# edawson/rkmh

Measured on AMD Instinct MI355X. Metric: reads classified/sec, higher is better.
Workload: dtype u64; 1 GPU; stream (C2): 1000000 synthetic 150 bp reads per GPU vs data/all_pave_ref.fa (182 refs), k=16 s=1000; reads_per_gpu=1000000, read_len=150, k=16, sketch_size=1000, references=182, parallelism=reads sharded over 1 rank(s); ref sketches RCCL-broadcast once

## Files before the change

### rkmh_amd/csrc/rk_kmer.hip

```cpp
#include "rk_kernels.hpp"

#include <cstdlib>
#include <type_traits>

namespace rk {

namespace {

constexpr int KW = 64;
constexpr int KM_MAX_T = 8;
constexpr int KM_MQ = 32;
constexpr int KM_CH = 2;
constexpr int KM_QCAP = 64 + 4 * KW;
constexpr int KM_LDS_SMALL = 5120;
constexpr int KM_LDS_BIG = 20480;
constexpr int KM_WAVES = 8;

enum { CM_DENSE8 = 0, CM_DENSE16 = 1, CM_SPARSE = 2 };

struct KmerGeom {
    int32_t T;
    int32_t cwords;
    int32_t dset;
    int32_t xcd;
    int32_t nmin_cap;
    int32_t L;
    int32_t gpr[KM_MAX_KS];
    uint32_t magic[KM_MAX_KS];
};

typedef uint32_t u32x4 __attribute__((ext_vector_type(4)));
struct __attribute__((packed, aligned(1))) km_pair1 { uint32_t x, y; };
struct __attribute__((packed, aligned(4))) km_pair4 { uint32_t x, y; };

template <int NQ>
struct KmLds {
    static constexpr int PK = 0;
    static constexpr int INV = PK + NQ * 64 + 2;
    static constexpr int Q = INV + NQ * 32 + 2;
    static constexpr int MQ = Q + KM_QCAP;
    static constexpr int RI = MQ + 2 * KM_MQ;
    static constexpr int NZ = RI + 4 * (KM_MAX_T + 1);
    static constexpr int BEST = NZ + KM_MAX_T;
    static constexpr int FLAGS = BEST + KM_MAX_T;
    static constexpr int NWT = FLAGS + KM_MAX_T;
    static constexpr int FAM = NWT + KM_MAX_T;
    static constexpr int FAMF = FAM + 4 * KM_MAX_T;
    static constexpr int CNT = FAMF + KM_MAX_T;
    static_assert(RI % 4 == 0, "rinfo is read with 16-byte LDS loads");
    static_assert(CNT % 4 == 0, "the multisets are cleared with 16-byte LDS stores");
};
inline size_t km_lds_bytes(const KmerGeom& g, int nq) {
    return ((size_t)(nq == 1 ? KmLds<1>::CNT : KmLds<2>::CNT) + (size_t)g.T * (size_t)(g.cwords + g.dset)) * 4;
}

__device__ __forceinline__ void wave_sync() {
    __builtin_amdgcn_fence(__ATOMIC_RELEASE, "wavefront");
    __builtin_amdgcn_wave_barrier();
    __builtin_amdgcn_fence(__ATOMIC_ACQUIRE, "wavefront");
}
template <int CTRL>
__device__ __forceinline__ int dpp_i32(int v) { return __builtin_amdgcn_update_dpp(v, v, CTRL, 0xf, 0xf, false); }
__device__ __forceinline__ int row_max_i32(int v) {
    int t;
    t = dpp_i32<0xB1>(v); v = t > v ? t : v;
    t = dpp_i32<0x4E>(v); v = t > v ? t : v;
    t = dpp_i32<0x141>(v); v = t > v ? t : v;
    t = dpp_i32<0x140>(v); v = t > v ? t : v;
    return v;
}
__device__ __forceinline__ int half_row_max_i32(int v) {
    int t;
    t = dpp_i32<0xB1>(v); v = t > v ? t : v;
    t = dpp_i32<0x4E>(v); v = t > v ? t : v;
    t = dpp_i32<0x141>(v); v = t > v ? t : v;
    return v;
}

__device__ __forceinline__ uint32_t km_pack4_hi(uint32_t x, uint32_t& mism) {
    const uint32_t c = (x >> 1) & 0x03030303u;
    mism |= (x & 0xDFDFDFDFu) ^ __builtin_amdgcn_perm(0x47544341u, 0x47544341u, c);
    return c * 0x01041040u;
}
__device__ __forceinline__ uint32_t km_pack16(const u32x4& v, uint32_t& mism) {
    const uint32_t m0 = km_pack4_hi(v.x, mism), m1 = km_pack4_hi(v.y, mism), m2 = km_pack4_hi(v.z, mism), m3 = km_pack4_hi(v.w, mism);
    const uint32_t lo = __builtin_amdgcn_perm(m1, m0, 0x0c0c0703u);
    const uint32_t hi = __builtin_amdgcn_perm(m3, m2, 0x07030c0cu);
    return lo | hi;
}
__device__ __forceinline__ uint32_t km_nonzero4(uint32_t m) {
    const uint32_t y = (m | ((m & 0x7f7f7f7fu) + 0x7f7f7f7fu)) & 0x80808080u;
    return ((y >> 7) * 0x01020408u) >> 24;
}

template <int CMODE>
__device__ __forceinline__ uint32_t km_field_max(uint32_t x) {
    if constexpr (CMODE == CM_DENSE8) {
        const uint32_t m01 = max(x & 0xFFu, (x >> 8) & 0xFFu), m23 = max((x >> 16) & 0xFFu, x >> 24);
        return max(m01, m23);
    } else return max(x & 0xFFFFu, x >> 16);
}

template <int KT, int NQ, int CMODE, bool BIG, bool FAM>
__global__ __launch_bounds__(KW, BIG ? 2 : KM_WAVES) void k_classify_kmer(const uint8_t* __restrict__ bases, const uint32_t* __restrict__ offs,
                                                                              uint32_t nreads, int S, RefIndex ix, KmerSets ksets,
                                                                              int32_t* __restrict__ out4, DevPolicy pol, KmerGeom geo) {
    static_assert(KT == 0 || KT == 32 || (KT >= 4 && KT <= 16), "a k-mer packs into 32 bits; the core is the (k-3)-mer");
    constexpr bool WIDE = KT == 32;
    using L = KmLds<NQ>;
    __shared__ __attribute__((aligned(16))) uint32_t smem[(BIG ? KM_LDS_BIG : KM_LDS_SMALL) / 4];
    constexpr uint32_t PAD_P = NQ * 1024;
    constexpr uint32_t clg = CMODE == CM_DENSE8 ? 2 : 1, cbits = 32u >> clg, cmask = (1u << cbits) - 1u;
    uint32_t* const pk = smem + L::PK;
    uint32_t* const inv = smem + L::INV;
    uint32_t* const q = smem + L::Q;
    uint32_t* const mq = smem + L::MQ;
    uint4* const rinfo = reinterpret_cast<uint4*>(smem + L::RI);
    uint32_t* const nzero = smem + L::NZ;
    uint32_t* const best = smem + L::BEST;
    uint32_t* const flags = smem + L::FLAGS;
    uint32_t* const nwtot = smem + L::NWT;
    uint32_t* const fam = smem + L::FAM;
    uint32_t* const famf = smem + L::FAMF;
    uint32_t* const cnt = smem + L::CNT;
    const int T = geo.T;
    const uint32_t CW = (uint32_t)geo.cwords, DS = (uint32_t)geo.dset;
    uint32_t* const dset = cnt + (uint32_t)T * CW;
    const uint32_t ds_shift = 32u - (uint32_t)__builtin_ctz(DS);
    const int lane = threadIdx.x;

    for (uint32_t i = lane; i < ((uint32_t)T * CW) >> 2; i += KW) reinterpret_cast<uint4*>(cnt)[i] = make_uint4(0u, 0u, 0u, 0u);
    const uint32_t ntiles = (nreads + (uint32_t)T - 1) / (uint32_t)T;
    const uintptr_t gb = reinterpret_cast<uintptr_t>(bases);
    const uintptr_t safe_hi = (gb + (uintptr_t)offs[nreads] + 4u) & ~(uintptr_t)3;

    auto tile_reads = [&](uint32_t tl) -> int {
        const uint32_t r = tl * (uint32_t)T;
        return (int)((nreads - r) < (uint32_t)T ? (nreads - r) : (uint32_t)T);
    };
    auto load_offsets = [&](uint32_t tl, uint32_t& a_, uint32_t& b_, uint32_t& o_) {
        const uint32_t r = tl * (uint32_t)T;
        const int n = tile_reads(tl);
        a_ = offs[r];
        b_ = offs[r + (uint32_t)n];
        o_ = offs[r + (uint32_t)(lane <= n ? lane : n)];
    };
    u32x4 pf[NQ];
    auto fetch_tile = [&](uint32_t a_, uint32_t b_) {
        const uintptr_t first = gb + a_;
        const uintptr_t base16 = first & ~(uintptr_t)15;
        const uint32_t nbytes = (uint32_t)(first - base16) + (b_ - a_);
        uint32_t nq = (nbytes + 15u) >> 4;
        if (nq > (uint32_t)(NQ * KW)) nq = NQ * KW;
        const bool safe = base16 >= gb && base16 + 16u * (uintptr_t)nq <= safe_hi;
#pragma unroll
        for (int r = 0; r < NQ; ++r) {
            const uint32_t qi = (uint32_t)r * KW + (uint32_t)lane;
            u32x4 v = {0u, 0u, 0u, 0u};
            if (qi < nq) {
                const uintptr_t qa = base16 + 16u * (uintptr_t)qi;
                if (safe) {
                    typedef const u32x4 __attribute__((address_space(1))) * gq_t;
                    v = __builtin_nontemporal_load((gq_t)qa);
                }
                else {
                    uint32_t d[4];
#pragma unroll
                    for (int j = 0; j < 4; ++j) {
                        const uintptr_t da = qa + 4u * (uintptr_t)j;
                        d[j] = (da >= gb && da + 4u <= safe_hi) ? *reinterpret_cast<const uint32_t*>(da) : 0u;
                    }
                    v.x = d[0]; v.y = d[1]; v.z = d[2]; v.w = d[3];
                }
            }
            pf[r] = v;
        }
    };

    uint32_t tile = blockIdx.x;
    if (geo.xcd) { const uint32_t per = (gridDim.x + 7u) >> 3; tile = (blockIdx.x & 7u) * per + (blockIdx.x >> 3); }
    if (tile >= ntiles) return;
    uint32_t cur_a = 0, cur_b = 0, cur_o = 0;
    load_offsets(tile, cur_a, cur_b, cur_o);
    fetch_tile(cur_a, cur_b);
    {
        const uint32_t r0 = tile * (uint32_t)T;
        const uint32_t ta = (uint32_t)__builtin_amdgcn_readfirstlane((int)cur_a);
        const uint32_t tb = (uint32_t)__builtin_amdgcn_readfirstlane((int)cur_b);
        const uint32_t mis = (uint32_t)((gb + ta) & 15u);
        const uint32_t nbytes = mis + (tb - ta);
        const uint32_t o_next = (uint32_t)__shfl_down((int)cur_o, 1);
        const uint32_t len = o_next - cur_o;
        int Tn = tile_reads(tile);
        uint32_t nq = (nbytes + 15u) >> 4;
        if (nbytes > (uint32_t)(NQ * 1024)) {
            const int Tn0 = Tn;
            Tn = __popcll(__ballot(lane < Tn0 && o_next - ta + mis <= (uint32_t)(NQ * 1024)));
            if (lane >= Tn && lane < Tn0) reinterpret_cast<int4*>(out4)[r0 + lane] = make_int4(-2, 0, 0, 0);
            nq = NQ * KW;
        }

        constexpr int NKC = KT ? 1 : KM_MAX_KS;
        const int NK = KT ? 1 : ksets.n;
        uint32_t nw_all = 0;
        if (lane < Tn) {
#pragma unroll
            for (int j = 0; j < NKC; ++j) if (j < NK) nw_all += (uint32_t)num_windows((int)len, WIDE ? (int)ix.kpk : (KT ? KT : ksets.k[j]), pol.drop_last_window);
        }
        if constexpr (FAM) { if (lane < 4 * KM_MAX_T) fam[lane] = 0; }
        if (lane < KM_MAX_T) {
            nzero[lane] = 0; best[lane] = 0; nwtot[lane] = nw_all;
            if constexpr (FAM) famf[lane] = 0;
            flags[lane] = nw_all > (CMODE == CM_SPARSE ? 0x7FFu : cmask) ? 1u : 0u;
        }
        const uint32_t ulen = (uint32_t)__builtin_amdgcn_readfirstlane((int)len);
        const bool same_len = __ballot(lane < Tn && len != ulen) == 0ull;
        uint32_t mism = 0;
#pragma unroll
        for (int r = 0; r < NQ; ++r) {
            const uint32_t qi = (uint32_t)r * KW + (uint32_t)lane;
            uint32_t m = 0;
            pk[qi] = km_pack16(pf[r], m);
            if (qi < nq) mism |= m;
        }
        if (lane < 2) pk[NQ * KW + lane] = 0;
        const bool has_invalid = __ballot(mism != 0u) != 0ull;
        if (has_invalid) {
#pragma unroll
            for (int r = 0; r < NQ; ++r) {
                const uint32_t qi = (uint32_t)r * KW + (uint32_t)lane;
                uint32_t m0 = 0, m1 = 0, m2 = 0, m3 = 0;
                km_pack4_hi(pf[r].x, m0); km_pack4_hi(pf[r].y, m1); km_pack4_hi(pf[r].z, m2); km_pack4_hi(pf[r].w, m3);
                const uint32_t b16 = km_nonzero4(m0) | (km_nonzero4(m1) << 4) | (km_nonzero4(m2) << 8) | (km_nonzero4(m3) << 12);
                reinterpret_cast<uint16_t*>(inv)[qi] = (uint16_t)(qi < nq ? b16 : 0u);
            }
            if (lane < 2) inv[NQ * 32 + lane] = 0;
        }
        for (int kk = 0; kk < NK; ++kk) {
        const int k = WIDE ? (int)ix.kpk : (KT ? KT : ksets.k[kk]);
        const uint32_t KMASK = (WIDE || k == 16) ? 0xffffffffu : ((1u << (2 * k)) - 1u);
        const uint32_t CMASK = WIDE ? 0xffffffffu : (1u << (2 * (k - 3))) - 1u;
        const uint64_t KMASK64 = WIDE ? (1ull << (2 * k)) - 1ull : 0ull, CMASK64 = WIDE ? (1ull << (2 * (k - 3))) - 1ull : 0ull;
        const uint32_t KBITS = (1u << k) - 1u;
        const uint4* const kf4p = KT ? ix.kf4 : ksets.kf4[kk];
        const uint4* const km1p = KT ? ix.km1 : ksets.km1[kk];
        const uint32_t* const km1v = KT ? ix.km1_vals : ksets.km1_vals[kk];
        const uint32_t kf4_n = KT ? ix.kf4_n : ksets.kf4_n[kk], km1_b = KT ? ix.km1_b : ksets.km1_b[kk];
        wave_sync();
        uint32_t nw = 0, ng = 0;
        if (lane < Tn) { nw = (uint32_t)num_windows((int)len, k, pol.drop_last_window); ng = (nw + 3u) >> 2; }
        uint32_t gs = ng;
        gs += (uint32_t)__builtin_amdgcn_update_dpp(0, (int)gs, 0x111, 0xf, 0xf, true);
        gs += (uint32_t)__builtin_amdgcn_update_dpp(0, (int)gs, 0x112, 0xf, 0xf, true);
        gs += (uint32_t)__builtin_amdgcn_update_dpp(0, (int)gs, 0x114, 0xf, 0xf, true);
        const uint32_t NG = (uint32_t)__builtin_amdgcn_readlane((int)gs, KM_MAX_T - 1);
        if (lane <= KM_MAX_T) rinfo[lane] = make_uint4(cur_o - ta + mis, nw, gs - ng, 0u);
        {
            uint4* d4 = reinterpret_cast<uint4*>(dset);
            for (uint32_t i = lane; i < ((uint32_t)Tn * DS) >> 2; i += KW) d4[i] = make_uint4(0u, 0u, 0u, 0u);
        }
        wave_sync();

        const uint32_t nw_u = (uint32_t)num_windows((int)ulen, k, pol.drop_last_window), gpr_u = (nw_u + 3u) >> 2;
        const bool uniform = same_len && gpr_u >= 2u;
        uint32_t magic = 0;
        if (uniform) magic = ulen == (uint32_t)geo.L ? geo.magic[kk] : (uint32_t)__builtin_amdgcn_readfirstlane((int)(0xFFFFFFFFu / gpr_u + 1u));
        uint32_t magic_v = magic, dlen_v = ulen - 4u * gpr_u;
        asm volatile("" : "+v"(magic_v), "+v"(dlen_v));

        auto count_posting = [&](uint32_t t, uint32_t crow_b, uint32_t ref) -> uint32_t {
            uint32_t* crow = reinterpret_cast<uint32_t*>(reinterpret_cast<uint8_t*>(cnt) + crow_b);
            const uint32_t M1 = CW - 1u, key = ref + 1u;
            uint32_t idx = ((ref * 0x9E3779B1u) >> 16) & M1, probe = 0, c = 0;
            for (; probe <= M1; ++probe) {
                const uint32_t old = atomicCAS(&crow[idx], 0u, (key << 11) | 1u);
                if (old == 0u) { c = 1u; break; }
                if ((old >> 11) == key) { c = (atomicAdd(&crow[idx], 1u) & 0x7FFu) + 1u; break; }
                idx = (idx + 1u) & M1;
            }
            if (probe > M1) { flags[t] = 1; return 0u; }
            return (c << 16) + (0xFFFFu - ref);
        };
        auto add_posting = [&](uint32_t t, uint32_t crow_b, uint32_t ref) {
            if constexpr (CMODE == CM_SPARSE) {
                const uint32_t v = count_posting(t, crow_b, ref);
                if (v) atomicMax(&best[t], v);
            } else {
                const uint32_t sh = (ref << (5 - clg)) & (32u - cbits);
                const uint32_t woff = (ref >> clg) << 2;
                atomicAdd(reinterpret_cast<uint32_t*>(reinterpret_cast<uint8_t*>(cnt) + crow_b + woff), 1u << sh);
            }
        };
        uint32_t mqn = 0;
        auto process_mq = [&]() {
            wave_sync();
            const uint32_t g = (uint32_t)lane >> 4, sl = (uint32_t)lane & 15u;
            auto walk = [&](uint32_t tr, const uint32_t* lp, uint32_t hdr, const km_pair4& pm0) {
                const uint32_t t = tr & 0xFFu, n = hdr & 0xFFFFFFu, base = FAM ? hdr >> 24 : 0u;
                if (base) {
                    if ((tr >> 8) != 0u) return;
                    if (sl == 0) { atomicAdd(&fam[4u * t + ((base - 1u) >> 1)], 1u << (16u * ((base - 1u) & 1u))); famf[t] = 1u; }
                    for (uint32_t c0 = 0; c0 < n; c0 += 16) {
                        const uint32_t c = c0 + sl;
                        if (c < n) {
                            km_pair4 pm = pm0;
                            if (c0) pm = *reinterpret_cast<const km_pair4*>(lp + 1 + 2 * c);
                            const uint32_t sh = (pm.x << (5 - clg)) & (32u - cbits), woff = (pm.x >> clg) << 2;
                            atomicAdd(reinterpret_cast<uint32_t*>(reinterpret_cast<uint8_t*>(cnt) + __umul24(t, CW * 4u) + woff), (pm.y >> 31) ? 0u - (1u << sh) : 1u << sh);
                        }
                    }
                    return;
                }
                for (uint32_t c0 = 0; c0 < n; c0 += 16) {
                    const uint32_t c = c0 + sl;
                    uint32_t v = 0;
                    if (c < n) {
                        km_pair4 pm = pm0;
                        if (c0) pm = *reinterpret_cast<const km_pair4*>(lp + 1 + 2 * c);
                        if ((tr >> 8) < pm.y) {
                            if constexpr (CMODE == CM_SPARSE) v = count_posting(t, __umul24(t, CW * 4u), pm.x);
                            else add_posting(t, __umul24(t, CW * 4u), pm.x);
                        }
                    }
                    if constexpr (CMODE == CM_SPARSE) {
                        v = (uint32_t)row_max_i32((int)v);
                        if (sl == 0 && v) atomicMax(&best[t], v);
                    }
                }
            };
            uint32_t j = g;
            uint32_t tr = 0, n = 0;
            const uint32_t* lp = ix.kpost;
            km_pair4 pm0{0u, 0u};
            if (j < mqn) { tr = mq[2 * j]; lp = ix.kpost + mq[2 * j + 1]; n = lp[0]; pm0 = *reinterpret_cast<const km_pair4*>(lp + 1 + 2 * sl); }
            while (j < mqn) {
                const uint32_t jn = j + KW / 16;
                uint32_t trn = 0, nn = 0;
                const uint32_t* lpn = ix.kpost;
                km_pair4 pmn{0u, 0u};
                if (jn < mqn) { trn = mq[2 * jn]; lpn = ix.kpost + mq[2 * jn + 1]; nn = lpn[0]; pmn = *reinterpret_cast<const km_pair4*>(lpn + 1 + 2 * sl); }
                walk(tr, lp, n, pm0);
                j = jn; tr = trn; lp = lpn; n = nn; pm0 = pmn;
            }
            wave_sync();
            mqn = 0;
        };
        struct Cand { uint32_t key, t, y, key_hi; uint4 c; };
        const uint32_t km_r = WIDE ? 8u : 2u * (uint32_t)k - km1_b, km_vb1 = 32u - KM1_HB - km_r;
        const uint32_t km_vmask = (1u << (km_vb1 - 1u)) - 1u, km_rmask = (1u << km_r) - 1u, nref = (uint32_t)ix.nref;
        auto wide_probe = [&](const Cand& c, const uint4& b, uint32_t hop, uint3& res, bool& again) {
            const uint32_t want = (hop << KW_TAG) | (c.y & ((1u << KW_TAG) - 1u));
            const uint32_t cells[4] = {b.x, b.y, b.z, b.w};
            res = make_uint3(KW_VID_NONE, 0u, 0u);
#pragma unroll
            for (int q = 0; q < 4; ++q) {
                const uint32_t num = cells[q] & KW_EMPTY;
                if ((cells[q] >> (KW_IDBITS + 1)) == want && num != KW_EMPTY && res.x == KW_VID_NONE) {
                    const uint2 kk = ix.kkeys[num];
                    if (kk.x == c.key && (kk.y & 0xFFu) == c.key_hi) res = make_uint3(kk.y >> 8, 0u, num);
                }
            }
            again = res.x == KW_VID_NONE && ((b.w >> KW_IDBITS) & 1u) != 0u && c.t != 0xFFFFFFFFu;
        };
        auto lookup = [&](uint32_t e, uint32_t qn) -> Cand {
            Cand c;
            uint32_t ent = PAD_P | (8u << 12);
            if (e < qn) ent = q[e];
            const uint32_t P = ent & 4095u, t = ent >> 12;
            const km_pair1 w = *reinterpret_cast<const km_pair1*>(reinterpret_cast<const uint8_t*>(pk) + (P >> 2));
            const uint2 ri = *reinterpret_cast<const uint2*>(&rinfo[t]);
            c.t = P - ri.x < ri.y ? t : 0xFFFFFFFFu;
            if constexpr (WIDE) {
                const uint64_t x = (join64(w.x, w.y) >> ((P & 3u) << 1)) & KMASK64;
                const uint64_t r = packed_revcomp64(x, k);
                const uint64_t key = x < r ? x : r;
                c.key = (uint32_t)key; c.key_hi = (uint32_t)(key >> 32);
                c.y = (uint32_t)(kw_y(key, k) >> (2u * (uint32_t)k - km1_b - KW_TAG));
                c.c = km1p[c.y >> KW_TAG];
                return c;
            }
            const uint32_t x = __builtin_amdgcn_alignbit(w.y, w.x, (P & 3u) << 1) & KMASK;
            const uint32_t r = packed_revcomp(x, k);
            c.key = x < r ? x : r;
            c.key_hi = 0;
            c.y = km1_y(c.key, k);
            c.c = km1p[c.y >> km_r];
            return c;
        };
        auto match_cell = [&](const uint4& b, uint32_t wantsh) -> uint32_t {
            const uint32_t lim = 1u << km_vb1;
            return (b.x ^ wantsh) < lim ? b.x : ((b.y ^ wantsh) < lim ? b.y : ((b.z ^ wantsh) < lim ? b.z : ((b.w ^ wantsh) < lim ? b.w : 0xFFFFFFFFu)));
        };
        auto first_match = [&](const Cand& c, uint32_t& cell, bool& again) {
            cell = match_cell(c.c, (c.y & km_rmask) << km_vb1);
            again = (cell & km_vmask) == km_vmask && ((c.c.w >> (km_vb1 - 1u)) & 1u) != 0u && c.t != 0xFFFFFFFFu;
        };
        auto hop_load = [&](const Cand& c, uint32_t hop, bool again) -> u32x4 {
            u32x4 v = {0u, 0u, 0u, 0u};
            if (again) v = *reinterpret_cast<const u32x4*>(km1p + (((c.y >> km_r) + hop) & ((1u << km1_b) - 1u)));
            return v;
        };
        auto next_match = [&](const Cand& c, uint32_t hop, const u32x4& nv, uint32_t& cell, bool& again) {
            if (again) {
                const uint4 nb = make_uint4(nv.x, nv.y, nv.z, nv.w);
                cell = match_cell(nb, ((c.y & km_rmask) << km_vb1) | (hop << (32u - KM1_HB)));
                again = (cell & km_vmask) == km_vmask && ((nb.w >> (km_vb1 - 1u)) & 1u) != 0u;
            }
        };
        auto apply = [&](const Cand& c, uint32_t cell, uint3 wres = make_uint3(0u, 0u, 0u)) {
            uint32_t vid = cell & km_vmask;
            bool hit = vid != km_vmask && c.t != 0xFFFFFFFFu;
            bool zero = vid == km_vmask - 1u;
            if constexpr (WIDE) {
                vid = wres.x;
                hit = vid != KW_VID_NONE && c.t != 0xFFFFFFFFu;
                zero = vid == KW_VID_ZERO;
                if (hit && !zero && ix.keepkey) { const uint32_t kid = ix.kslots[wres.z]; if (!((ix.keepkey[kid >> 5] >> (kid & 31u)) & 1u)) zero = true; }
            }
            uint32_t val = vid | (1u << 20);
            uint32_t valy = 0, valz = 0, valw = 0;
            if (hit && vid >= nref && !zero) {
                const uint4 vv = *reinterpret_cast<const uint4*>(km1v + 4u * (vid - nref));
                val = vv.x; valy = vv.y; valz = vv.z; valw = vv.w;
                if constexpr (CMODE == CM_SPARSE) { if ((val >> 29) == 7u) val = 0x80000000u | valz; }
            }
            uint32_t rank = 0;
            bool multi = false;
            if (hit) {
                if (zero) atomicAdd(&nzero[c.t], 1u);
                else {
                    uint32_t* ds = dset + c.t * DS;
                    const uint32_t id = (WIDE ? wres.z : c.key) + 1u;
                    uint32_t idx = ((id - 1u) * 0x9E3779B1u) >> ds_shift;
                    uint32_t old = atomicCAS(&ds[idx], 0u, id);
                    uint32_t probes = 1;
                    while (old != 0u && probes < DS) {
                        rank += old == id ? 1u : 0u;
                        idx = (idx + 1u) & (DS - 1u);
                        old = atomicCAS(&ds[idx], 0u, id);
                        ++probes;
                    }
                    if (old != 0u) flags[c.t] = 1;
                    else if (FAM && (val >> 29) == 7u) {
                        if (rank == 0) {
                            const uint32_t base = (val >> 26) & 7u, nex = (val >> 22) & 15u, crow_b = __umul24(c.t, CW * 4u);
                            atomicAdd(&fam[4u * c.t + (base >> 1)], 1u << (16u * (base & 1u)));
                            famf[c.t] = 1u;
                            auto signed_add = [&](uint32_t f) {
                                const uint32_t ref = f & 511u, sh = (ref << (5 - clg)) & (32u - cbits);
                                atomicAdd(reinterpret_cast<uint32_t*>(reinterpret_cast<uint8_t*>(cnt) + crow_b + ((ref >> clg) << 2)), (f & 512u) ? 0u - (1u << sh) : 1u << sh);
                            };
                            if (nex > 0u) signed_add(val & 1023u);
                            if (nex > 1u) signed_add((val >> 10) & 1023u);
                            if (nex > 2u) signed_add(valy & 1023u);
                            if (nex > 3u) signed_add((valy >> 10) & 1023u);
                            if (nex > 4u) signed_add((valy >> 20) & 1023u);
                            if (nex > 5u) signed_add(valw & 1023u);
                            if (nex > 6u) signed_add((valw >> 10) & 1023u);
                            if (nex > 7u) signed_add((valw >> 20) & 1023u);
                        }
                    }
                    else if ((val >> 30) == 3u || !(val >> 31)) {
                        const bool three = (val >> 30) == 3u, two = !three && ((val >> 29) & 3u) != 0u;
                        const uint32_t fw = three ? 9u : 11u;
                        const uint32_t lim = (three || two) ? 1u : ((val >> 20) & 0x1FFu);
                        const uint32_t n = rank >= lim ? 0u : (three ? 3u + ((val >> 27) & 3u) : (two ? 2u : 1u));
                        const uint32_t refs[6] = {__builtin_amdgcn_ubfe(val, 0u, three ? 9u : (two ? 11u : 20u)), __builtin_amdgcn_ubfe(val, fw, fw),
                                                  (val >> 18) & 511u, valy & 511u, (valy >> 9) & 511u, (valy >> 18) & 511u};
                        const uint32_t crow_b = __umul24(c.t, CW * 4u);
#pragma unroll
                        for (uint32_t j = 0; j < 6u; ++j) if (j < n) add_posting(c.t, crow_b, refs[j]);
                    } else multi = true;
                }
            }
            const uint32_t listoff = (CMODE == CM_SPARSE ? valz : val) & 0x3fffffffu;
            uint64_t mm = __ballot(multi);
            while (mm) {
                const uint32_t pos = __builtin_amdgcn_mbcnt_hi((uint32_t)(mm >> 32), __builtin_amdgcn_mbcnt_lo((uint32_t)mm, 0u));
                const uint32_t space = (uint32_t)KM_MQ - mqn;
                if (multi && pos < space) {
                    mq[2 * (mqn + pos)] = c.t | (rank << 8); mq[2 * (mqn + pos) + 1] = listoff;
                    multi = false;
                }
                const uint32_t tot = (uint32_t)__popcll(mm);
                mqn += tot < space ? tot : space;
                if (mqn == (uint32_t)KM_MQ) process_mq();
                mm = __ballot(multi);
            }
        };
        auto drain = [&](uint32_t qn) {
            for (uint32_t e0 = 0; e0 < qn; e0 += 2 * KW) {
                const bool two = e0 + KW < qn;
                const Cand a = lookup(e0 + (uint32_t)lane, qn);
                Cand b{0u, 0xFFFFFFFFu, 0u, 0u, make_uint4(0u, 0u, 0u, 0u)};
                if (two) b = lookup(e0 + KW + (uint32_t)lane, qn);
                if constexpr (WIDE) {
                    uint3 ra, rb = make_uint3(KW_VID_NONE, 0u, 0u);
                    bool ga, gb = false;
                    wide_probe(a, a.c, 0u, ra, ga);
                    if (two) wide_probe(b, b.c, 0u, rb, gb);
                    for (uint32_t hop = 1; hop < (1u << KM1_HB) && __ballot(ga || gb); ++hop) {
                        const uint32_t bm = (1u << km1_b) - 1u;
                        if (ga) { const uint4 nb = km1p[((a.y >> KW_TAG) + hop) & bm]; wide_probe(a, nb, hop, ra, ga); }
                        if (gb) { const uint4 nb = km1p[((b.y >> KW_TAG) + hop) & bm]; wide_probe(b, nb, hop, rb, gb); }
                    }
                    apply(a, 0u, ra);
                    if (two) apply(b, 0u, rb);
                    continue;
                }
                uint32_t ca, cb = 0xFFFFFFFFu;
                bool ga, gb = false;
                first_match(a, ca, ga);
                if (two) first_match(b, cb, gb);
                for (uint32_t hop = 1; hop < (1u << KM1_HB) && __ballot(ga || gb); ++hop) {
                    u32x4 na = hop_load(a, hop, ga), nb = hop_load(b, hop, gb);
                    asm volatile("" : "+v"(na), "+v"(nb));
                    next_match(a, hop, na, ca, ga);
                    next_match(b, hop, nb, cb, gb);
                }
                apply(a, ca);
                if (two) apply(b, cb);
            }
            if (mqn) process_mq();
        };

        const uint32_t nsteps = (NG + KW - 1) / KW;
        const bool qlast = !WIDE && NG != 0u && ((NG - 1u) & (uint32_t)(KW - 1)) < 16u;
        const uint32_t kf4_n16 = kf4_n << 4;
        uint32_t qcount = 0;
        uint32_t step = 0;
        for (;;) {
            uint32_t wl[KM_CH], wh[KM_CH], e0v[KM_CH], fq[KM_CH];
            u32x4 fw[KM_CH];
            bool isqv[KM_CH];
#pragma unroll
            for (int s = 0; s < KM_CH; ++s) {
                const bool isq = qlast && step + (uint32_t)s + 1u == nsteps;
                isqv[s] = isq;
                const uint32_t jq = isq ? (uint32_t)lane & 3u : 0u;
                const uint32_t G = (step + (uint32_t)s) * KW + (isq ? (uint32_t)lane >> 2 : (uint32_t)lane);
                uint32_t t, P0;
                if (uniform) {
                    t = __umulhi(G, magic_v);
                    P0 = __umul24(t, dlen_v) + ((G << 2) + mis);
                } else {
                    t = 0;
#pragma unroll
                    for (int i = 1; i < KM_MAX_T; ++i) t += G >= rinfo[i].z ? 1u : 0u;
                    const uint4 ri = rinfo[t];
                    P0 = ri.x + 4u * (G - ri.z);
                }
                const bool act = G < NG;
                if (!act) { P0 = PAD_P; t = 8u; }
                const km_pair1 w = *reinterpret_cast<const km_pair1*>(reinterpret_cast<const uint8_t*>(pk) + (P0 >> 2));
                const uint32_t sh = (P0 & 3u) << 1;
                wl[s] = __builtin_amdgcn_alignbit(w.y, w.x, sh);
                wh[s] = w.y >> sh;
                uint32_t core = k == 16 ? wl[s] >> 6 : (wl[s] >> 6) & CMASK;
                if constexpr (WIDE) core = kw_fold((join64(wl[s], wh[s]) >> 6) & CMASK64);
                const uint32_t sect_b = __umulhi(core * 0x85EBCA6Bu, kf4_n16) & ~15u;
                e0v[s] = P0 | (t << 12);
                fq[s] = 0u;
                fw[s] = u32x4{0u, 0u, 0u, 0u};
                if (isq) {
                    wl[s] = __builtin_amdgcn_alignbit(wh[s], wl[s], 2u * jq);
                    if (act) e0v[s] += jq;
                    fq[s] = *reinterpret_cast<const uint32_t*>(reinterpret_cast<const uint8_t*>(kf4p) + (sect_b + 4u * jq));
                } else fw[s] = *reinterpret_cast<const u32x4*>(reinterpret_cast<const uint8_t*>(kf4p) + sect_b);
            }
            bool stop = false;
            uint32_t done = 0;
            auto test_step = [&](int s, auto inv_tag, auto nw_tag) {
                constexpr bool INV = decltype(inv_tag)::value;
                constexpr int NW = decltype(nw_tag)::value;
                uint32_t ib = 0, nz = 0, nwt = 0, t_ = 0, o0 = 0;
                bool act = true;
                if constexpr (INV) {
                    const uint32_t P0 = e0v[s] & 4095u;
                    t_ = e0v[s] >> 12;
                    act = t_ != 8u;
                    if (act) {
                        ib = __builtin_amdgcn_alignbit(inv[(P0 >> 5) + 1], inv[P0 >> 5], P0 & 31u);
                        const uint2 ri = *reinterpret_cast<const uint2*>(&rinfo[t_]);
                        nwt = ri.y; o0 = P0 - ri.x;
                    }
                }
#pragma unroll
                for (int j = 0; j < NW; ++j) {
                    uint32_t x = j == 0 ? wl[s] : __builtin_amdgcn_alignbit(wh[s], wl[s], 2 * j);
                    if (k < 16) x &= KMASK;
                    if constexpr (WIDE) x = kw_fold((join64(wl[s], wh[s]) >> (2 * j)) & KMASK64);
                    const uint32_t f = NW == 1 ? fq[s] : (j == 0 ? fw[s].x : (j == 1 ? fw[s].y : (j == 2 ? fw[s].z : fw[s].w)));
                    const uint32_t fb = kf4_bits_dev(x);
                    bool cand = (fb & f) == fb;
                    if constexpr (INV) {
                        if (act && ((ib >> j) & KBITS) != 0u) {
                            cand = false;
                            if (o0 + (uint32_t)j < nwt) ++nz;
                        }
                    }
                    const uint64_t m = __builtin_amdgcn_ballot_w64(cand);
                    if (__builtin_amdgcn_inverse_ballot_w64(m)) {
                        const uint32_t mb = __builtin_amdgcn_mbcnt_hi((uint32_t)(m >> 32), __builtin_amdgcn_mbcnt_lo((uint32_t)m, 0u));
                        *reinterpret_cast<uint32_t*>(reinterpret_cast<uint8_t*>(q) + ((mb << 2) + (qcount << 2))) = e0v[s] + (uint32_t)j;
                    }
                    qcount += (uint32_t)__builtin_popcountll(m);
                }
                if constexpr (INV) { if (nz) atomicAdd(&nzero[t_], nz); }
            };
#pragma unroll
            for (int s = 0; s < KM_CH; ++s) {
                if (step + (uint32_t)s < nsteps && !stop) {
                    if (qcount + 4u * KW > (uint32_t)KM_QCAP) stop = true;
                    else {
                        ++done;
                        if (isqv[s]) {
                            if (has_invalid) test_step(s, std::true_type{}, std::integral_constant<int, 1>{});
                            else test_step(s, std::false_type{}, std::integral_constant<int, 1>{});
                        } else if (has_invalid) test_step(s, std::true_type{}, std::integral_constant<int, 4>{});
                        else test_step(s, std::false_type{}, std::integral_constant<int, 4>{});
                    }
                }
            }
            step += done;
            const bool last = step >= nsteps;
            wave_sync();
            const uint32_t qn = last ? qcount : (qcount & ~(uint32_t)(KW - 1));
            drain(qn);
            wave_sync();
            if (last) break;
            const uint32_t rem = qcount - qn;
            uint32_t ce = 0;
            if ((uint32_t)lane < rem) ce = q[qn + lane];
            wave_sync();
            if ((uint32_t)lane < rem) q[lane] = ce;
            qcount = rem;
            wave_sync();
        }

        }
        wave_sync();

        {
            const int lsh = Tn > 4 ? 3 : 4, LPR = 1 << lsh;
            const int g = lane >> lsh, sl = lane & (LPR - 1);
            for (int t = g; t < Tn; t += KW >> lsh) {
                uint32_t* ct = cnt + (uint32_t)t * CW;
                const int nmins = (int)nwtot[t] - (int)nzero[t];
                const bool reroute = nmins > S || flags[t] != 0;
                if (reroute) {
                    if (sl == 0) reinterpret_cast<int4*>(out4)[r0 + t] = make_int4(-2, 0, 0, 0);
                    continue;
                }
                if constexpr (FAM && CMODE != CM_SPARSE) {
                    if (famf[t]) {
                        for (uint32_t b = 0; b < 8u; ++b) {
                            const uint32_t h = (fam[4u * (uint32_t)t + (b >> 1)] >> (16u * (b & 1u))) & 0xFFFFu;
                            if (h == 0u) continue;
                            const uint32_t start = ix.kbase[2u * b], nm = ix.kbase[2u * b + 1u];
                            for (uint32_t m0 = 0; m0 < nm; m0 += (uint32_t)LPR) {
                                const uint32_t m = m0 + (uint32_t)sl;
                                if (m < nm) {
                                    const uint32_t ref = ix.kbase[start + m];
                                    atomicAdd(&ct[ref >> clg], h << ((ref << (5 - clg)) & (32u - cbits)));
                                }
                            }
                        }
                        __builtin_amdgcn_fence(__ATOMIC_RELEASE, "wavefront");
                        __builtin_amdgcn_fence(__ATOMIC_ACQUIRE, "wavefront");
                    }
                }
                int max_id, max_shared, prev;
                if constexpr (CMODE == CM_SPARSE) {
                    const uint32_t bk = best[t];
                    max_id = bk ? (int)(0xFFFFu - (bk & 0xFFFFu)) : 0;
                    max_shared = (int)(bk >> 16);
                    prev = max_id > 0 ? 0 : -1;
                    for (uint32_t w = sl; w < CW; w += LPR) {
                        const uint32_t x = ct[w];
                        const int r_ = (int)(x >> 11) - 1, cj = (int)(x & 0x7FFu);
                        if (x != 0u && r_ < max_id && cj > prev) prev = cj;
                    }
                } else {
                    const uint32_t nwl = (CW + (uint32_t)LPR - 1u) >> lsh, wbase = (uint32_t)sl * nwl;
                    uint32_t lmax = 0, lpre = 0, lfirst = wbase;
                    for (uint32_t i = 0; i < nwl; ++i) {
                        const uint32_t w = wbase + i;
                        const uint32_t m = km_field_max<CMODE>(ct[w < CW ? w : CW - 1u]);
                        if (m > lmax) { lpre = lmax; lmax = m; lfirst = w; }
                    }
                    const uint32_t lkey = (lmax << 8) | (255u - lfirst);
                    const uint32_t km = (uint32_t)(LPR == 16 ? row_max_i32((int)lkey) : half_row_max_i32((int)lkey));
                    const uint32_t M = km >> 8, wb = 255u - (km & 255u);
                    const uint32_t xb = ct[wb];
                    const uint32_t ones = CMODE == CM_DENSE8 ? 0x01010101u : 0x00010001u;
                    const uint32_t y = xb ^ (M * ones);
                    const uint32_t z = (y - ones) & ~y & (ones << (cbits - 1u));
                    const uint32_t qf = (uint32_t)__builtin_ctz(z) >> (5 - clg);
                    max_id = M ? (int)((wb << clg) + qf) : 0;
                    max_shared = (int)M;
                    uint32_t acc = km_field_max<CMODE>(__builtin_amdgcn_ubfe(xb, 0u, qf << (5 - clg)));
                    if (lkey == km) acc = max(acc, lpre);
                    else if (wbase + nwl <= wb) acc = max(acc, lmax);
                    prev = max_id > 0 ? (int)acc : -1;
                }
                prev = LPR == 16 ? row_max_i32(prev) : half_row_max_i32(prev);
                if (sl == 0) reinterpret_cast<int4*>(out4)[r0 + t] = make_int4(max_id, max_shared, max_shared - prev, nmins < geo.nmin_cap ? nmins : geo.nmin_cap);
            }
        }
    }
}

bool make_kmer_geom(KmerGeom& g, int maxlen, int nref, int expect_hits, int win_total, const int* nw_k, int nk, int nq, int& cmode, bool& big) {
    if (maxlen < 1) maxlen = 1;
    cmode = win_total <= 255 ? CM_DENSE8 : CM_DENSE16;
    const int clg = cmode == CM_DENSE8 ? 2 : 1;
    g.cwords = (nref + (1 << clg) - 1) >> clg;
    if (nref > 0 && g.cwords >= 129) { cmode = CM_SPARSE; g.cwords = 128; }
    g.cwords = (g.cwords + 3) & ~3;
    int ds = 64;
    while (ds < 3 * expect_hits && ds < 1024) ds <<= 1;
    g.dset = ds;
    int T = (nq * 1024 - 15) / maxlen;
    if (T > KM_MAX_T) T = KM_MAX_T;
    if (T < 1) T = 1;
    g.T = T;
    big = false;
    while (g.T > 1 && km_lds_bytes(g, nq) > (size_t)KM_LDS_SMALL) g.T -= 1;
    if (km_lds_bytes(g, nq) > (size_t)KM_LDS_SMALL || 2 * g.T < T) {
        big = true;
        g.T = T;
        while (g.T > 1 && km_lds_bytes(g, nq) > (size_t)KM_LDS_BIG) g.T -= 1;
        if (km_lds_bytes(g, nq) > (size_t)KM_LDS_BIG) return false;
    }
    g.xcd = 1;
    g.L = maxlen;
    for (int j = 0; j < KM_MAX_KS; ++j) {
        g.gpr[j] = j < nk ? (nw_k[j] + 3) >> 2 : 0;
        g.magic[j] = g.gpr[j] >= 2 ? 0xFFFFFFFFu / (uint32_t)g.gpr[j] + 1u : 0u;
    }
    return true;
}

template <int KT>
hipError_t launch_k(int nq, int cmode, bool big, bool fam, dim3 grid, hipStream_t st, const uint8_t* bases, const uint32_t* offs, uint32_t nreads,
                    int S, const RefIndex& ix, const KmerSets& ksets, int32_t* out4, const DevPolicy& pol, const KmerGeom& geo) {
#define RK_KM_GO(NQ, CM, BIG, FAM) hipLaunchKernelGGL((k_classify_kmer<KT, NQ, CM, BIG, FAM>), grid, dim3(KW), 0, st, bases, offs, nreads, S, ix, ksets, out4, pol, geo)
#define RK_KM_CM(NQ, BIG)                                                                                    \
    do {                                                                                                     \
        if (cmode == CM_DENSE8) { if (fam) RK_KM_GO(NQ, CM_DENSE8, BIG, true); else RK_KM_GO(NQ, CM_DENSE8, BIG, false); } \
        else if (cmode == CM_DENSE16) { if (fam) RK_KM_GO(NQ, CM_DENSE16, BIG, true); else RK_KM_GO(NQ, CM_DENSE16, BIG, false); } \
        else RK_KM_GO(NQ, CM_SPARSE, BIG, true);                                                             \
    } while (0)
    if (nq == 1 && !big) RK_KM_CM(1, false);
    else if (nq == 1) RK_KM_CM(1, true);
    else if (!big) RK_KM_CM(2, false);
    else RK_KM_CM(2, true);
#undef RK_KM_CM
#undef RK_KM_GO
    return hipGetLastError();
}

}

bool classify_kmer_supported(int nref, int maxlen, int k) {
    return nref <= 16384 && maxlen <= 2 * 1024 - 15 && k >= KPRE_MIN_K && k <= KW_MAX_K;
}

hipError_t launch_classify_kmer(const uint8_t* bases, const uint32_t* offs, uint32_t nreads, const KmerSets& ksets, int S, const RefIndex& ix,
                                int32_t* out4, const DevPolicy& pol, int maxlen, int expect_hits, hipStream_t st, int nmin_cap) {
    if (nreads == 0) return hipSuccess;
    if (ksets.n < 1 || ksets.n > KM_MAX_KS) return hipErrorInvalidValue;
    const int nq = maxlen <= 1024 - 15 ? 1 : 2;
    int nw_k[KM_MAX_KS] = {0}, win_total = 0;
    for (int j = 0; j < ksets.n; ++j) { nw_k[j] = num_windows(maxlen, ksets.k[j], pol.drop_last_window); win_total += nw_k[j]; }
    KmerGeom geo;
    int cmode = 0;
    bool big = false;
    if (!make_kmer_geom(geo, maxlen, ix.nref, expect_hits, win_total, nw_k, ksets.n, nq, cmode, big)) return hipErrorInvalidConfiguration;
    geo.nmin_cap = nmin_cap;
    const uint32_t ntiles = (nreads + (uint32_t)geo.T - 1) / (uint32_t)geo.T;
    const bool fam = ix.kbase_n != 0u;
    uint32_t grid = ntiles;
    grid = (grid + 7u) & ~7u;
    if (ksets.n > 1) return launch_k<0>(nq, cmode, big, fam, dim3(grid), st, bases, offs, nreads, S, ix, ksets, out4, pol, geo);
#define RK_KM_K(KT) case KT: return launch_k<KT>(nq, cmode, big, fam, dim3(grid), st, bases, offs, nreads, S, ix, ksets, out4, pol, geo)
    switch (ksets.k[0]) {
        RK_KM_K(8); RK_KM_K(9); RK_KM_K(10); RK_KM_K(11); RK_KM_K(12); RK_KM_K(13); RK_KM_K(14); RK_KM_K(15); RK_KM_K(16);
        case 17: case 18: case 19: case 20:
            return ix.kkeys ? launch_k<32>(nq, cmode, big, fam, dim3(grid), st, bases, offs, nreads, S, ix, ksets, out4, pol, geo) : hipErrorInvalidValue;
        default: return hipErrorInvalidValue;
    }
#undef RK_KM_K
}

}
```

Measured before the change: 3.354 billion reads/s.

## Software-pipeline k-mer window loads and defer queue overflow via pending masks

Replaces the fixed two-step chunk loop with a software-pipelined loop that issues the packed-sequence and filter loads for the next step while testing the current one. Instead of stopping early when the queue might overflow by a worst-case bound, it computes the exact ballot counts and, on overflow, saves the candidate bits as pending to push after the drain. Uniform/invalid variants are specialised at compile time. This aims to hide global-load latency and cut the number of drains, at the cost of more complex control flow and higher register pressure.

```diff
diff --git a/rkmh_amd/csrc/rk_kmer.hip b/rkmh_amd/csrc/rk_kmer.hip
--- a/rkmh_amd/csrc/rk_kmer.hip
+++ b/rkmh_amd/csrc/rk_kmer.hip
@@ -10,7 +10,6 @@
 constexpr int KW = 64;
 constexpr int KM_MAX_T = 8;
 constexpr int KM_MQ = 32;
-constexpr int KM_CH = 2;
 constexpr int KM_QCAP = 64 + 4 * KW;
 constexpr int KM_LDS_SMALL = 5120;
 constexpr int KM_LDS_BIG = 20480;
@@ -526,104 +525,140 @@
 
         const uint32_t nsteps = (NG + KW - 1) / KW;
         const bool qlast = !WIDE && NG != 0u && ((NG - 1u) & (uint32_t)(KW - 1)) < 16u;
+        const uint32_t nfull = nsteps - (qlast ? 1u : 0u);
         const uint32_t kf4_n16 = kf4_n << 4;
         uint32_t qcount = 0;
         uint32_t step = 0;
+        bool pending = false;
+        uint32_t pend_e0 = 0, pend_c = 0;
+        struct Iss { uint32_t wl, wh, e0; u32x4 fw; };
+        auto issue = [&](uint32_t st, auto uni_tag, auto q_tag) -> Iss {
+            constexpr bool UNI = decltype(uni_tag)::value;
+            constexpr bool ISQ = decltype(q_tag)::value;
+            const uint32_t jq = ISQ ? (uint32_t)lane & 3u : 0u;
+            const uint32_t G = st * KW + (ISQ ? (uint32_t)lane >> 2 : (uint32_t)lane);
+            uint32_t t, P0;
+            if constexpr (UNI) {
+                t = __umulhi(G, magic_v);
+                P0 = __umul24(t, dlen_v) + ((G << 2) + mis);
+            } else {
+                t = 0;
+#pragma unroll
+                for (int i = 1; i < KM_MAX_T; ++i) t += G >= rinfo[i].z ? 1u : 0u;
+                const uint4 ri = rinfo[t];
+                P0 = ri.x + 4u * (G - ri.z);
+            }
+            const bool act = G < NG;
+            if (!act) { P0 = PAD_P; t = 8u; }
+            const km_pair1 w = *reinterpret_cast<const km_pair1*>(reinterpret_cast<const uint8_t*>(pk) + (P0 >> 2));
+            const uint32_t sh = (P0 & 3u) << 1;
+            Iss r;
+            r.wl = __builtin_amdgcn_alignbit(w.y, w.x, sh);
+            r.wh = w.y >> sh;
+            uint32_t core = k == 16 ? r.wl >> 6 : (r.wl >> 6) & CMASK;
+            if constexpr (WIDE) core = kw_fold((join64(r.wl, r.wh) >> 6) & CMASK64);
+            const uint32_t sect_b = __umulhi(core * 0x85EBCA6Bu, kf4_n16) & ~15u;
+            r.e0 = P0 | (t << 12);
+            if constexpr (ISQ) {
+                r.wl = __builtin_amdgcn_alignbit(r.wh, r.wl, 2u * jq);
+                if (act) r.e0 += jq;
+                r.fw = u32x4{*reinterpret_cast<const uint32_t*>(reinterpret_cast<const uint8_t*>(kf4p) + (sect_b + 4u * jq)), 0u, 0u, 0u};
+            } else r.fw = *reinterpret_cast<const u32x4*>(reinterpret_cast<const uint8_t*>(kf4p) + sect_b);
+            return r;
+        };
+        auto push = [&](uint32_t e0, uint64_t m, uint32_t j) {
+            if (__builtin_amdgcn_inverse_ballot_w64(m)) {
+                const uint32_t mb = __builtin_amdgcn_mbcnt_hi((uint32_t)(m >> 32), __builtin_amdgcn_mbcnt_lo((uint32_t)m, 0u));
+                *reinterpret_cast<uint32_t*>(reinterpret_cast<uint8_t*>(q) + ((mb << 2) + (qcount << 2))) = e0 + j;
+            }
+            qcount += (uint32_t)__builtin_popcountll(m);
+        };
+        auto test = [&](const Iss& c, auto inv_tag, auto nw_tag) -> bool {
+            constexpr bool INV = decltype(inv_tag)::value;
+            constexpr int NW = decltype(nw_tag)::value;
+            uint32_t ib = 0, nz = 0, nwt = 0, t_ = 0, o0 = 0;
+            bool act = true;
+            if constexpr (INV) {
+                const uint32_t P0 = c.e0 & 4095u;
+                t_ = c.e0 >> 12;
+                act = t_ != 8u;
+                if (act) {
+                    ib = __builtin_amdgcn_alignbit(inv[(P0 >> 5) + 1], inv[P0 >> 5], P0 & 31u);
+                    const uint2 ri = *reinterpret_cast<const uint2*>(&rinfo[t_]);
+                    nwt = ri.y; o0 = P0 - ri.x;
+                }
+            }
+            uint64_t m[NW];
+            uint32_t tot = 0;
+#pragma unroll
+            for (int j = 0; j < NW; ++j) {
+                uint32_t x = j == 0 ? c.wl : __builtin_amdgcn_alignbit(c.wh, c.wl, 2 * j);
+                if (k < 16) x &= KMASK;
+                if constexpr (WIDE) x = kw_fold((join64(c.wl, c.wh) >> (2 * j)) & KMASK64);
+                const uint32_t f = j == 0 ? c.fw.x : (j == 1 ? c.fw.y : (j == 2 ? c.fw.z : c.fw.w));
+                const uint32_t fb = kf4_bits_dev(x);
+                bool cand = (fb & f) == fb;
+                if constexpr (INV) {
+                    if (act && ((ib >> j) & KBITS) != 0u) {
+                        cand = false;
+                        if (o0 + (uint32_t)j < nwt) ++nz;
+                    }
+                }
+                m[j] = __builtin_amdgcn_ballot_w64(cand);
+                tot += (uint32_t)__builtin_popcountll(m[j]);
+            }
+            if constexpr (INV) { if (nz) atomicAdd(&nzero[t_], nz); }
+            if (qcount + tot > (uint32_t)KM_QCAP) {
+                pend_e0 = c.e0; pend_c = 0;
+#pragma unroll
+                for (int j = 0; j < NW; ++j) pend_c |= __builtin_amdgcn_inverse_ballot_w64(m[j]) ? 1u << j : 0u;
+                pending = true;
+                return false;
+            }
+#pragma unroll
+            for (int j = 0; j < NW; ++j) push(c.e0, m[j], (uint32_t)j);
+            return true;
+        };
+        auto windows = [&](auto uni_tag, auto inv_tag) {
+            const std::true_type quarter{}; const std::false_type full{};
+            const std::integral_constant<int, 4> w4{}; const std::integral_constant<int, 1> w1{};
+            if (pending) {
+#pragma unroll
+                for (uint32_t j = 0; j < 4u; ++j) push(pend_e0, __builtin_amdgcn_ballot_w64(((pend_c >> j) & 1u) != 0u), j);
+                pending = false;
+            }
+            if (step >= nsteps) return;
+            if (step == nfull) {
+                const Iss cq = issue(step, uni_tag, quarter);
+                ++step;
+                test(cq, inv_tag, w1);
+                return;
+            }
+            Iss cur = issue(step, uni_tag, full);
+            while (step + 1u < nfull) {
+                const Iss nxt = issue(step + 1u, uni_tag, full);
+                ++step;
+                if (!test(cur, inv_tag, w4)) return;
+                cur = nxt;
+            }
+            if (qlast) {
+                const Iss cq = issue(step + 1u, uni_tag, quarter);
+                ++step;
+                if (!test(cur, inv_tag, w4)) return;
+                ++step;
+                test(cq, inv_tag, w1);
+            } else {
+                ++step;
+                test(cur, inv_tag, w4);
+            }
+        };
         for (;;) {
-            uint32_t wl[KM_CH], wh[KM_CH], e0v[KM_CH], fq[KM_CH];
-            u32x4 fw[KM_CH];
-            bool isqv[KM_CH];
-#pragma unroll
-            for (int s = 0; s < KM_CH; ++s) {
-                const bool isq = qlast && step + (uint32_t)s + 1u == nsteps;
-                isqv[s] = isq;
-                const uint32_t jq = isq ? (uint32_t)lane & 3u : 0u;
-                const uint32_t G = (step + (uint32_t)s) * KW + (isq ? (uint32_t)lane >> 2 : (uint32_t)lane);
-                uint32_t t, P0;
-                if (uniform) {
-                    t = __umulhi(G, magic_v);
-                    P0 = __umul24(t, dlen_v) + ((G << 2) + mis);
-                } else {
-                    t = 0;
-#pragma unroll
-                    for (int i = 1; i < KM_MAX_T; ++i) t += G >= rinfo[i].z ? 1u : 0u;
-                    const uint4 ri = rinfo[t];
-                    P0 = ri.x + 4u * (G - ri.z);
-                }
-                const bool act = G < NG;
-                if (!act) { P0 = PAD_P; t = 8u; }
-                const km_pair1 w = *reinterpret_cast<const km_pair1*>(reinterpret_cast<const uint8_t*>(pk) + (P0 >> 2));
-                const uint32_t sh = (P0 & 3u) << 1;
-                wl[s] = __builtin_amdgcn_alignbit(w.y, w.x, sh);
-                wh[s] = w.y >> sh;
-                uint32_t core = k == 16 ? wl[s] >> 6 : (wl[s] >> 6) & CMASK;
-                if constexpr (WIDE) core = kw_fold((join64(wl[s], wh[s]) >> 6) & CMASK64);
-                const uint32_t sect_b = __umulhi(core * 0x85EBCA6Bu, kf4_n16) & ~15u;
-                e0v[s] = P0 | (t << 12);
-                fq[s] = 0u;
-                fw[s] = u32x4{0u, 0u, 0u, 0u};
-                if (isq) {
-                    wl[s] = __builtin_amdgcn_alignbit(wh[s], wl[s], 2u * jq);
-                    if (act) e0v[s] += jq;
-                    fq[s] = *reinterpret_cast<const uint32_t*>(reinterpret_cast<const uint8_t*>(kf4p) + (sect_b + 4u * jq));
-                } else fw[s] = *reinterpret_cast<const u32x4*>(reinterpret_cast<const uint8_t*>(kf4p) + sect_b);
-            }
-            bool stop = false;
-            uint32_t done = 0;
-            auto test_step = [&](int s, auto inv_tag, auto nw_tag) {
-                constexpr bool INV = decltype(inv_tag)::value;
-                constexpr int NW = decltype(nw_tag)::value;
-                uint32_t ib = 0, nz = 0, nwt = 0, t_ = 0, o0 = 0;
-                bool act = true;
-                if constexpr (INV) {
-                    const uint32_t P0 = e0v[s] & 4095u;
-                    t_ = e0v[s] >> 12;
-                    act = t_ != 8u;
-                    if (act) {
-                        ib = __builtin_amdgcn_alignbit(inv[(P0 >> 5) + 1], inv[P0 >> 5], P0 & 31u);
-                        const uint2 ri = *reinterpret_cast<const uint2*>(&rinfo[t_]);
-                        nwt = ri.y; o0 = P0 - ri.x;
-                    }
-                }
-#pragma unroll
-                for (int j = 0; j < NW; ++j) {
-                    uint32_t x = j == 0 ? wl[s] : __builtin_amdgcn_alignbit(wh[s], wl[s], 2 * j);
-                    if (k < 16) x &= KMASK;
-                    if constexpr (WIDE) x = kw_fold((join64(wl[s], wh[s]) >> (2 * j)) & KMASK64);
-                    const uint32_t f = NW == 1 ? fq[s] : (j == 0 ? fw[s].x : (j == 1 ? fw[s].y : (j == 2 ? fw[s].z : fw[s].w)));
-                    const uint32_t fb = kf4_bits_dev(x);
-                    bool cand = (fb & f) == fb;
-                    if constexpr (INV) {
-                        if (act && ((ib >> j) & KBITS) != 0u) {
-                            cand = false;
-                            if (o0 + (uint32_t)j < nwt) ++nz;
-                        }
-                    }
-                    const uint64_t m = __builtin_amdgcn_ballot_w64(cand);
-                    if (__builtin_amdgcn_inverse_ballot_w64(m)) {
-                        const uint32_t mb = __builtin_amdgcn_mbcnt_hi((uint32_t)(m >> 32), __builtin_amdgcn_mbcnt_lo((uint32_t)m, 0u));
-                        *reinterpret_cast<uint32_t*>(reinterpret_cast<uint8_t*>(q) + ((mb << 2) + (qcount << 2))) = e0v[s] + (uint32_t)j;
-                    }
-                    qcount += (uint32_t)__builtin_popcountll(m);
-                }
-                if constexpr (INV) { if (nz) atomicAdd(&nzero[t_], nz); }
-            };
-#pragma unroll
-            for (int s = 0; s < KM_CH; ++s) {
-                if (step + (uint32_t)s < nsteps && !stop) {
-                    if (qcount + 4u * KW > (uint32_t)KM_QCAP) stop = true;
-                    else {
-                        ++done;
-                        if (isqv[s]) {
-                            if (has_invalid) test_step(s, std::true_type{}, std::integral_constant<int, 1>{});
-                            else test_step(s, std::false_type{}, std::integral_constant<int, 1>{});
-                        } else if (has_invalid) test_step(s, std::true_type{}, std::integral_constant<int, 4>{});
-                        else test_step(s, std::false_type{}, std::integral_constant<int, 4>{});
-                    }
-                }
-            }
-            step += done;
-            const bool last = step >= nsteps;
+            if (uniform) {
+                if (has_invalid) windows(std::true_type{}, std::true_type{});
+                else windows(std::true_type{}, std::false_type{});
+            } else if (has_invalid) windows(std::false_type{}, std::true_type{});
+            else windows(std::false_type{}, std::false_type{});
+            const bool last = !pending;
             wave_sync();
             const uint32_t qn = last ? qcount : (qcount & ~(uint32_t)(KW - 1));
             drain(qn);
```

After: 3.345 billion reads/s. About the same (-0.3%).
